# ISU-PAAL/DeepDFA

Measured on NVIDIA H100. Metric: CFG graphs/sec (train step), higher is better.
Workload: dtype f32 (GRU GEMMs: bf16x3 split operands, f32 accumulate)

## Files before the change

### deepdfa_b200/_lib.py

```python
from __future__ import annotations

import ctypes as C
import os
import re
from pathlib import Path

from . import build as _build

HEADER = Path(__file__).resolve().parent.parent / "include" / "ddfa_b200.h"

ENGINE_SIMT = 0
ENGINE_TCGEN05 = 1


class DdfaError(RuntimeError):
    pass


def declared_symbols():
    text = HEADER.read_text()
    text = re.sub(r"/\*.*?\*/", "", text, flags=re.S)
    return sorted(set(re.findall(r"\b(ddfa_[a-z0-9_]+)\s*\(", text)))


# ... 34 lines not shown
    "ddfa_gru_step_fwd_image_v2": (_int, [_vp, _vp, _vp, _vp, _i32, _i32, _vp, _vp, _vp, _vp, _sz, _vp]),
    "ddfa_gru_step_bwd_image_v2": (_int, [_vp] * 9 + [_i32, _i32] + [_vp] * 7 + [_vp, _sz, _int, _vp]),
    "ddfa_gru_step_bwd_image": (_int, [_vp] * 9 + [_i32, _i32] + [_vp] * 7 + [_vp, _sz, _int, _vp]),
    "ddfa_gru_step_bwd_finish": (_int, [_i32, _i32, _vp, _vp, _vp, _sz, _vp]),
    "ddfa_gru_step_bwd_workspace_bytes": (_sz, [_i32, _i32, _int]),
    "ddfa_gru_step_bwd_workspace_bytes_steps": (_sz, [_i32, _i32, _int, _i32]),
    "ddfa_gru_bwd_wgrad_batched": (_int, [_vp, _vp, _i32, _i32, _i32, _vp, _vp, _vp, _sz, _vp]),
    "ddfa_gru_step_prepare_bwd": (_int, [_vp, _vp, _i32, _int, _vp, _sz, _vp]),
    "ddfa_gru_step_bwd": (_int, [_vp] * 7 + [_i32, _i32] + [_vp] * 7 + [_vp, _sz, _int, _vp]),
    "ddfa_ggnn_workspace_bytes": (_sz, [_i32, _i32, _i32, _int, _int]),
    "ddfa_ggnn_fwd": (_int, [_vp, _vp, _vp, _i32, _i32, _i32] + [_vp] * 7 + [_vp, _sz, _int, _int, _vp]),
    "ddfa_ggnn_bwd": (_int, [_vp, _vp, _vp, _vp, _i32, _i32, _i32] + [_vp] * 12 + [_vp, _sz, _int, _vp]),
    "ddfa_readout_mlp_fwd": (_int, [_vp, _vp, _vp, _i32, _i32, _vp, _vp, _vp, _vp, _i32] + [_vp] * 6 + [_vp]),
    "ddfa_mlp_bwd": (_int, [_vp, _vp, _vp, _vp, _i32, _i32, _i32, _vp, _vp, _vp, _vp, _vp]),
    "ddfa_readout_bwd": (_int, [_vp] * 5 + [_i32, _i32] + [_vp] * 8 + [_vp]),
    "ddfa_graph_label_bce": (_int, [_vp, _vp, _vp, _i32, _f32, _f32, _f32, _vp, _vp, _vp, _vp]),
    "ddfa_graph_label_bce_valid": (_int, [_vp, _vp, _vp, _i32, _i32, _f32, _f32, _f32, _vp, _vp, _vp, _vp]),
    "ddfa_adam_flat": (_int, [_vp, _vp, _vp, _vp, _vp, _i64, _f32, _f32, _f32, _f32, _f32, _vp]),
    "ddfa_allreduce_adam_p2p": (_int, [_vp, _vp, _vp, _i32, _i32, _vp, _vp, _vp, _i64, _i64, _vp, _vp, _f32, _f32, _f32, _f32, _f32, _vp]),
    "ddfa_sgemm": (_int, [_int, _int, _i32, _i32, _i32, _f32, _vp, _i32, _vp, _i32, _f32, _vp, _i32, _i32, _vp]),
}

TUNE_L2_HINTS, TUNE_PDL_MASK, TUNE_GATHER_VARIANT, TUNE_FWD_PAIR, TUNE_GATE_BWD_TMA, TUNE_GATHER_SRC_GROUPS = 0, 1, 2, 3, 4, 5

_NO_STATUS = {"ddfa_gru_gates_packed_bytes", "ddfa_tuning_get", "ddfa_abi_version", "ddfa_last_error", "ddfa_device_supported", "ddfa_launch_count", "ddfa_engine_available",
              "ddfa_build_csr_workspace_bytes", "ddfa_arena_batch_workspace_bytes", "ddfa_gru_step_workspace_bytes", "ddfa_gru_step_bwd_workspace_bytes", "ddfa_gru_step_bwd_workspace_bytes_steps",
              "ddfa_act_image_bytes", "ddfa_ggnn_workspace_bytes"}


class _Lib:
    def __init__(self):
        path = Path(os.environ["DDFA_LIB_PATH"]) if os.environ.get("DDFA_LIB_PATH") else _build.LIB
        if not path.exists():
            raise DdfaError(
                f"{path} is missing: build it with `python -m deepdfa_b200.build` (or __graft_entry__.build()). "
                "deepdfa_b200 has no CPU / PyTorch fallback.")
        self.path = path
        self._dll = C.CDLL(str(path))
        missing = []
        for name, (res, args) in _SIGNATURES.items():
            try:
                fn = getattr(self._dll, name)
            except AttributeError:
                missing.append(name)
                continue
            fn.restype = res
            fn.argtypes = args
        if missing:
            raise DdfaError(f"{path} does not export: {missing}")
        abi = self._dll.ddfa_abi_version()
        if abi != 1:
            raise DdfaError(f"ABI version mismatch: library {abi}, binding 1")
        for env, key in (("DDFA_L2_HINTS", TUNE_L2_HINTS), ("DDFA_PDL", TUNE_PDL_MASK), ("DDFA_GATHER_VARIANT", TUNE_GATHER_VARIANT),
                         ("DDFA_GATE_BWD_TMA", TUNE_GATE_BWD_TMA),
                         ("DDFA_GATHER_SRC_GROUPS", TUNE_GATHER_SRC_GROUPS)):
            if os.environ.get(env) is not None:
                self._dll.ddfa_tuning_set(key, int(os.environ[env]))

    def last_error(self) -> str:
        msg = self._dll.ddfa_last_error()
        return msg.decode() if msg else ""

    def raw(self, name):
        return getattr(self._dll, name)

    def call(self, name, *args):
        rc = getattr(self._dll, name)(*args)
        if name not in _NO_STATUS and rc != 0:
            raise DdfaError(f"{name} failed (status {rc}): {self.last_error()}")
        return rc


_LIB = None


def lib() -> _Lib:
    global _LIB
    if _LIB is None:
# ... 8 lines not shown
```

### deepdfa_b200/csrc/abi.cu

```cuda
#include <stdarg.h>
#include <stdlib.h>
#include <string.h>

#include <atomic>

#include "common.cuh"

namespace ddfa {
static std::atomic<long long> g_launches{0};
void count_launch() { g_launches.fetch_add(1, std::memory_order_relaxed); }

static thread_local char g_err[512] = "";

static thread_local bool g_chain_break = true;
void chain_break() { g_chain_break = true; }
bool chain_take_break() {
  const bool b = g_chain_break;
  g_chain_break = false;
  return b;
}

static std::atomic<int> g_tuning[DDFA_TUNE__COUNT] = {
    {23},
    {15},
    {9},
    {0},
    {2},
    {0},
};
int l2_hints() { return g_tuning[DDFA_TUNE_L2_HINTS].load(std::memory_order_relaxed); }
int pdl_mask() { return g_tuning[DDFA_TUNE_PDL_MASK].load(std::memory_order_relaxed); }
int gather_variant() { return g_tuning[DDFA_TUNE_GATHER_VARIANT].load(std::memory_order_relaxed); }
int gate_bwd_tma() { return g_tuning[DDFA_TUNE_GATE_BWD_TMA].load(std::memory_order_relaxed); }
int gather_src_groups() { return g_tuning[DDFA_TUNE_GATHER_SRC_GROUPS].load(std::memory_order_relaxed); }

void set_error(const char *fmt, ...) {
  va_list ap;
  va_start(ap, fmt);
  vsnprintf(g_err, sizeof(g_err), fmt, ap);
  va_end(ap);
}
}

extern "C" {

int ddfa_abi_version(void) { return DDFA_ABI_VERSION; }

const char *ddfa_last_error(void) { return ddfa::g_err; }

int ddfa_engine_available(int engine) {
  if (engine == DDFA_ENGINE_SIMT) return 1;
  if (engine == DDFA_ENGINE_TCGEN05) return 1;
  return 0;
}

int ddfa_tuning_set(int key, int value) {
  DDFA_REQUIRE(key >= 0 && key < DDFA_TUNE__COUNT, "ddfa_tuning_set: unknown key %d", key);
  DDFA_REQUIRE(key != DDFA_TUNE_FWD_PAIR || value == 0, "ddfa_tuning_set: DDFA_TUNE_FWD_PAIR must be 0 (no CTA-pair forward kernel on sm_90a)");
  ddfa::g_tuning[key].store(value, std::memory_order_relaxed);
  return DDFA_OK;
}
int ddfa_tuning_get(int key) {
  if (key < 0 || key >= DDFA_TUNE__COUNT) return -1;
  return ddfa::g_tuning[key].load(std::memory_order_relaxed);
}

int ddfa_debug_set(int key, int value) {
  switch (key) {
    case 2: {
      int rc = ddfa::gru_tc3_trace_enable(value);
      return rc != DDFA_OK ? rc : ddfa::gru_tc2b_trace_enable(value);
    }
    default: ddfa::set_error("ddfa_debug_set: unknown key %d", key); return DDFA_ERR_INVALID_ARG;
  }
}

int ddfa_debug_read(int key, void *host_out, size_t bytes) {
  DDFA_REQUIRE(host_out != nullptr, "ddfa_debug_read: null output");
  switch (key) {
    case 2: return ddfa::gru_tc2b_trace_read(host_out, bytes);
    case 3: return ddfa::gru_tc3_trace_read(host_out, bytes);
// ... 23 lines not shown
```

### deepdfa_b200/csrc/common.cuh

```cuda
#pragma once
#include <cuda_runtime.h>
#include <stdint.h>
#include <stdio.h>

#include "../../include/ddfa_b200.h"

namespace ddfa {

void set_error(const char *fmt, ...);
void count_launch();

inline cudaStream_t as_stream(void *s) { return reinterpret_cast<cudaStream_t>(s); }

#define DDFA_REQUIRE(cond, ...)            \
  do {                                     \
    if (!(cond)) {                         \
      ddfa::set_error(__VA_ARGS__);        \
      return DDFA_ERR_INVALID_ARG;         \
    }                                      \
  } while (0)

#define DDFA_CHECK_LAUNCH(name)                                                        \
  do {                                                                                 \
    cudaError_t e__ = cudaGetLastError();                                              \
// ... 1 lines not shown
      ddfa::set_error("%s: launch failed: %s", name, cudaGetErrorString(e__));         \
      return DDFA_ERR_CUDA;                                                            \
    }                                                                                  \
    ddfa::count_launch();                                                              \
  } while (0)

#define DDFA_CUDA(call)                                                                \
  do {                                                                                 \
    cudaError_t e__ = (call);                                                          \
    if (e__ != cudaSuccess) {                                                          \
      ddfa::set_error("%s failed: %s", #call, cudaGetErrorString(e__));                \
      return DDFA_ERR_CUDA;                                                            \
    }                                                                                  \
  } while (0)

__device__ __forceinline__ void pdl_launch_dependents() { asm volatile("griddepcontrol.launch_dependents;" ::: "memory"); }
__device__ __forceinline__ void pdl_wait() { asm volatile("griddepcontrol.wait;" ::: "memory"); }
int pdl_mask();
int gather_variant();
int gather_src_groups();
int gate_bwd_tma();
void chain_break();
bool chain_take_break();

template <typename... KArgs, typename... Args>
inline cudaError_t launch_chain_cluster(int which, int cluster_x, void (*kernel)(KArgs...), dim3 grid, dim3 block, size_t smem,
                                        cudaStream_t stream, Args... args) {
  cudaLaunchConfig_t cfg = {};
  cfg.gridDim = grid;
  cfg.blockDim = block;
  cfg.dynamicSmemBytes = smem;
  cfg.stream = stream;
  cudaLaunchAttribute attr[2];
  int n = 0;
  if (cluster_x > 1) {
    attr[n].id = cudaLaunchAttributeClusterDimension;
    attr[n].val.clusterDim.x = (unsigned)cluster_x;
    attr[n].val.clusterDim.y = 1;
    attr[n].val.clusterDim.z = 1;
    ++n;
  }
  const bool brk = chain_take_break();
  if ((pdl_mask() & which) && !brk) {
    attr[n].id = cudaLaunchAttributeProgrammaticStreamSerialization;
    attr[n].val.programmaticStreamSerializationAllowed = 1;
    ++n;
// ... 131 lines not shown
```

### deepdfa_b200/csrc/gru_tc_bwd.cu

```cuda
#include <cuda_fp16.h>

#include "tc_common.cuh"

namespace ddfa {
namespace tc2b {
using namespace tcc;

constexpr int kThreads = 320, kEpiWarps = 8;

constexpr int kGbWarps = 8;
struct GbRow {
  float4 d, hv, rr, zz, nn, gh;
  float deg;
  int tb, te;
};
__device__ __forceinline__ float4 bf16x4_to_f4(const uint2 &p) {
  return make_float4(__uint_as_float(p.x << 16), __uint_as_float(p.x & 0xffff0000u), __uint_as_float(p.y << 16), __uint_as_float(p.y & 0xffff0000u));
}
__device__ __forceinline__ void gb_load(GbRow &x, const float *__restrict__ dh_out, const float *__restrict__ h,
                                        const uint8_t *__restrict__ h_img_src, const float *__restrict__ gates,
                                        const uint4 *__restrict__ gates_packed, const int32_t *__restrict__ indptr,
                                        const int32_t *__restrict__ indptr_t, size_t plane, int64_t node, int col, bool ok,
                                        uint64_t pol_saved, uint64_t pol_dh) {
  x.tb = x.te = 0;
// ... 465 lines not shown
        }
      }
    }
    wgmma_wait<0>();
    wgmma_fence_regs(acc);
    if (tr) { trace_stamp(tron, k, 6); trace_stamp(tron, k, 8); }
    __syncwarp();
    if (lane == 0) mbar_arrive(empty(pending));
    pending = -1;
    if (tr) trace_stamp(tron, k, 9);
#pragma unroll
    for (int hh = 0; hh < 2; ++hh) {
      const int64_t node = (int64_t)tile * kTileM + row0 + 8 * hh;
      if (node < N) {
#pragma unroll
        for (int j = 0; j < 8; ++j)
          st_f2_hint(out + node * kD + col0 + 8 * j, make_float2(acc[4 * j + 2 * hh] + dv[hh][j].x, acc[4 * j + 2 * hh + 1] + dv[hh][j].y), pol_tmp);
      }
    }
    if (tr) trace_stamp(tron, k, 10);
  }
}

constexpr int kWgSlotBytes = kImageTileBytes;
constexpr int kWgSlots = 3;
constexpr int kWgOffBar = kWgSlots * kWgSlotBytes;
constexpr int kWgSmemAlloc = kWgOffBar + 2 * kWgSlots * 8 + 1024;
constexpr int kWgThreads = 32 * kEpiWarps + 32;
constexpr size_t kWgPartialFloats = (size_t)3 * kD * kD;
constexpr int kWgMaxSteps = 16;
struct WgBatch {
  const uint8_t *s_img[kWgMaxSteps];
  const uint8_t *h_img[kWgMaxSteps];
  int32_t steps;
};
__global__ void __launch_bounds__(kWgThreads, 1) wgrad_kernel(const uint8_t *__restrict__ q_img, size_t img_stride, size_t step_stride,
                                                              const __grid_constant__ WgBatch batch,
                                                              int32_t N, float *__restrict__ partial, int first, int hints) {
  extern __shared__ uint8_t smem_raw[];
  uint8_t *smem = reinterpret_cast<uint8_t *>((reinterpret_cast<uintptr_t>(smem_raw) + 1023) & ~(uintptr_t)1023);
  const uint32_t sbase = smem_u32(smem);
  const uint32_t bar0 = sbase + kWgOffBar;
  auto full = [&](int i) { return bar0 + 8u * i; };
  auto empty = [&](int i) { return bar0 + 8u * (kWgSlots + i); };

  const int warp = threadIdx.x >> 5, lane = threadIdx.x & 31;
  const int role = blockIdx.y / 3, g = blockIdx.y % 3;
  const int qm = g < 2 ? g : (role == 0 ? 2 : 3);
  const int num_tiles = (N + kTileM - 1) / kTileM;
  const int all_tiles = num_tiles * batch.steps;
  const int my_tiles = (all_tiles > (int)blockIdx.x) ? (all_tiles - 1 - (int)blockIdx.x) / (int)gridDim.x + 1 : 0;

  if (threadIdx.x == 0) {
    for (int i = 0; i < kWgSlots; ++i) { mbar_init(full(i), 1); mbar_init(empty(i), kEpiWarps); }
    mbar_fence_init();
  }
  __syncthreads();
  const int tron = (g_trace_on == 2) && blockIdx.y == 0;
  if (threadIdx.x == 0) trace_stamp(tron, 0, 0);

  if (warp == kEpiWarps) {
    if (elect_one()) {
      const uint64_t pol_wg = l2_policy((hints & 32) ? 1 : 0);
      for (int i = 0; i < my_tiles; ++i) {
        const int idx = (int)blockIdx.x + i * (int)gridDim.x;
        const int t = idx / num_tiles, tile = idx - t * num_tiles;
        for (int w = 0; w < 2; ++w) {
          const int cc = 2 * i + w, slot = cc % kWgSlots, use = cc / kWgSlots;
          if (use > 0) mbar_wait_bounded(empty(slot), (use - 1) & 1);
          const uint8_t *src = w == 0 ? (role == 0 ? batch.s_img[t] : batch.h_img[t]) : q_img + (size_t)t * step_stride + (size_t)qm * img_stride;
          mbar_arrive_expect_tx(full(slot), kWgSlotBytes);
          bulk_g2s_hint(sbase + slot * kWgSlotBytes, src + (size_t)tile * kImageTileBytes, kWgSlotBytes, full(slot), pol_wg);
          trace_stamp(tron, i, 1 + w);
        }
      }
    }
    return;
  }

  const int wg = warp >> 2;
  float acc[64];
#pragma unroll
  for (int i = 0; i < 64; ++i) acc[i] = 0.f;
  for (int i = 0; i < my_tiles; ++i) {
    const int cb = 2 * i, ca = 2 * i + 1;
    mbar_wait_bounded(full(cb % kWgSlots), (cb / kWgSlots) & 1);
    if (warp == 0 && lane == 0) trace_stamp(tron, i, 3);
    mbar_wait_bounded(full(ca % kWgSlots), (ca / kWgSlots) & 1);
    if (warp == 0 && lane == 0) { trace_stamp(tron, i, 4); trace_stamp(tron, i, 5); }
    const uint32_t b0 = sbase + (cb % kWgSlots) * kWgSlotBytes;
    const uint32_t a0 = sbase + (ca % kWgSlots) * kWgSlotBytes + wg * kChunkBytes;
    constexpr uint32_t vs = 2 * kChunkBytes;
    wgmma_fence();
#pragma unroll
    for (int k16 = 0; k16 < kTileM / 16; ++k16) {
      const uint32_t koff = (uint32_t)k16 * 2048u;
      const uint64_t a_hi = gmma_desc(a0 + koff, kChunkBytes), a_lo = gmma_desc(a0 + vs + koff, kChunkBytes);
      const uint64_t b_hi = gmma_desc(b0 + koff, kChunkBytes), b_lo = gmma_desc(b0 + vs + koff, kChunkBytes);
      wgmma_n128<1, 1>(acc, a_hi, b_hi, 1u);
      wgmma_n128<1, 1>(acc, a_lo, b_hi, 1u);
      wgmma_n128<1, 1>(acc, a_hi, b_lo, 1u);
    }
    wgmma_commit();
    if (warp == 0 && lane == 0) trace_stamp(tron, i, 6);
    wgmma_wait<0>();
    __syncwarp();
    if (lane == 0) { mbar_arrive(empty(cb % kWgSlots)); mbar_arrive(empty(ca % kWgSlots)); }
  }
  wgmma_fence_regs(acc);
  if (warp == 0 && lane == 0) trace_stamp(tron, 0, 8);
  float *dst = partial + ((size_t)role * gridDim.x + blockIdx.x) * kWgPartialFloats;
  const int row0 = g * kD + wg * 64 + (warp & 3) * 16 + (lane >> 2);
#pragma unroll
  for (int hh = 0; hh < 2; ++hh) {
    float *rowp = dst + (size_t)(row0 + 8 * hh) * kD + 2 * (lane & 3);
#pragma unroll
    for (int j = 0; j < 16; ++j) {
      float2 v = make_float2(acc[4 * j + 2 * hh], acc[4 * j + 2 * hh + 1]);
      if (!first) {
        const float2 o = *reinterpret_cast<const float2 *>(rowp + 8 * j);
        v.x += o.x;
        v.y += o.y;
      }
      *reinterpret_cast<float2 *>(rowp + 8 * j) = v;
    }
  }
  if (warp == 0 && lane == 0) trace_stamp(tron, 0, 10);
}

__global__ void __launch_bounds__(256) wgrad_reduce_kernel(const float *__restrict__ partial, int ctas, float *__restrict__ dw_fold,
                                                           float *__restrict__ dw_hh) {
// ... 155 lines not shown
```

### deepdfa_b200/csrc/gru_tc_fwd3.cu

```cuda
#include <cuda_fp16.h>
#include <stdlib.h>

#include "tc_common.cuh"

namespace ddfa {
namespace tc3 {
using namespace tcc;

constexpr int kSlices = 4;
constexpr int kSliceCols = kD / kSlices;
constexpr int kRowsPerPart = 3 * kSliceCols;
constexpr int kWChunkBytes = kRowsPerPart * 128;
constexpr int kSliceWBytes = 8 * kWChunkBytes;
constexpr int kStageBytes = kImageTileBytes;
constexpr int kOffStage = kSliceWBytes;
constexpr int kOffBias = kOffStage + 2 * kStageBytes;
constexpr int kBiasSlice = 7 * kSliceCols;
constexpr int kOffBar = kOffBias + kBiasSlice * 4;
constexpr int kSmemAlloc = kOffBar + 5 * 8;
constexpr int kConsumerWarps = 8;
constexpr int kThreads = 32 * kConsumerWarps + 32;
constexpr size_t kPackedWBytes = (size_t)kSlices * kSliceWBytes;
constexpr size_t kPackedBytes = kPackedWBytes + (size_t)kSlices * kBiasSlice * 4;
static_assert(kSmemAlloc <= 232448, "shared memory budget");
// ... 11 lines not shown
  uint4 ph, pl;
  split8(x, ph, pl);
  uint8_t *base = packed + (size_t)slice * kSliceWBytes + sw128_offset(n, (u & 7) * 8);
  *reinterpret_cast<uint4 *>(base + ((p * 2 + 0) * 2 + kb) * kWChunkBytes) = ph;
  *reinterpret_cast<uint4 *>(base + ((p * 2 + 1) * 2 + kb) * kWChunkBytes) = pl;
  if (p == 0 && u == 0 && n < kSliceCols) {
    const int t = slice * kSliceCols + n;
    float *bias = reinterpret_cast<float *>(packed + kPackedWBytes) + slice * kBiasSlice;
    bias[0 * kSliceCols + n] = b_ih[2 * kD + t];
    bias[1 * kSliceCols + n] = b_ih[t] + b_hh[t];
    bias[2 * kSliceCols + n] = b_ih[kD + t] + b_hh[kD + t];
    bias[3 * kSliceCols + n] = b_hh[2 * kD + t];
    bias[4 * kSliceCols + n] = b_fold[2 * kD + t];
    bias[5 * kSliceCols + n] = b_fold[t];
    bias[6 * kSliceCols + n] = b_fold[kD + t];
  }
}

template <bool HIMG, int GATES>
__global__ void __launch_bounds__(kThreads, 1) gru_fwd3_kernel(const uint8_t *__restrict__ s_img, const uint8_t *__restrict__ h_img,
                                                               const float *__restrict__ h, const int32_t *__restrict__ indptr,
                                                               const uint8_t *__restrict__ packed, int32_t N,
                                                               float *__restrict__ h_out, uint8_t *__restrict__ h_out_img,
                                                               float *__restrict__ gates, uint2 *__restrict__ gates_packed, int hints) {
  extern __shared__ __align__(1024) uint8_t smem[];
  const uint32_t sbase = smem_u32(smem);
  if ((sbase & 1023u) != 0) __trap();
  const uint32_t bar0 = sbase + kOffBar;
  auto full = [&](int i) { return bar0 + 8u * i; };
  auto empty = [&](int i) { return bar0 + 8u * (2 + i); };
  const uint32_t w_full = bar0 + 32u;

  const int warp = threadIdx.x >> 5, lane = threadIdx.x & 31;
  const int slice = blockIdx.x % kSlices;
  const int group = blockIdx.x / kSlices, num_groups = gridDim.x / kSlices;
  const int num_tiles = (N + kTileM - 1) / kTileM;
  const int my_tiles = (num_tiles > group) ? (num_tiles - 1 - group) / num_groups + 1 : 0;

  if (threadIdx.x == 0) {
    for (int i = 0; i < 2; ++i) { mbar_init(full(i), 1); mbar_init(empty(i), kConsumerWarps); }
    mbar_init(w_full, 1);
    mbar_fence_init();
  }
  __syncthreads();
  const int tron = g_trace_on;
  if (threadIdx.x == 0) trace_stamp(tron, 0, 0);
  pdl_launch_dependents();

  if (warp == kConsumerWarps) {
    if (my_tiles > 0 && elect_one()) {
      mbar_arrive_expect_tx(w_full, kSliceWBytes);
      bulk_g2s(sbase, packed + (size_t)slice * kSliceWBytes, kSliceWBytes, w_full);
      pdl_wait();
      for (int k = 0; k < my_tiles; ++k) {
        const size_t toff = (size_t)(group + k * num_groups) * kImageTileBytes;
        for (int p = 0; p < 2; ++p) {
          if (k > 0) mbar_wait_bounded(empty(p), (k - 1) & 1);
          mbar_arrive_expect_tx(full(p), kStageBytes);
          bulk_g2s(sbase + kOffStage + p * kStageBytes, (p == 0 ? s_img : h_img) + toff, kStageBytes, full(p));
          trace_stamp(tron, k, 1 + p);
        }
      }
    }
    return;
  }

  float *sbias = reinterpret_cast<float *>(smem + kOffBias);
  for (int i = threadIdx.x; i < kBiasSlice; i += 32 * kConsumerWarps)
    sbias[i] = __ldcg(reinterpret_cast<const float *>(packed + kPackedWBytes) + slice * kBiasSlice + i);
  asm volatile("bar.sync 1, %0;" ::"n"(32 * kConsumerWarps) : "memory");
  pdl_wait();
  if (my_tiles == 0) return;
  const int wg = warp >> 2;
  const int row0 = wg * 64 + (warp & 3) * 16 + (lane >> 2);
  const int c4 = 2 * (lane & 3);
  const size_t plane = (size_t)N * kD;
  const uint64_t pol_gates = l2_policy((hints & 1) ? 1 : 0);
  const uint64_t pol_next = l2_policy((hints & 16) ? 2 : 0);
  mbar_wait_bounded(w_full, 0);
  const bool tr = (warp == 0 && lane == 0);

  for (int k = 0; k < my_tiles; ++k) {
    const int tile = group + k * num_groups;
    float acc_s[48], acc_h[48];
    if (tr) { trace_stamp(tron, k, 7); trace_stamp(tron, k, 3); }
    mbar_wait_bounded(full(0), k & 1);
    if (tr) trace_stamp(tron, k, 4);
    wgmma_fence();
#pragma unroll
    for (int p = 0; p < 2; ++p) {
      if (p == 1) {
        mbar_wait_bounded(full(1), k & 1);
        if (tr) trace_stamp(tron, k, 5);
      }
      const uint32_t a0 = sbase + kOffStage + p * kStageBytes + wg * 8192;
// ... 24 lines not shown
      const int64_t node = (int64_t)tile * kTileM + row0 + 8 * hh;
      const bool valid = node < N;
      deg[hh] = valid ? (float)(__ldcg(indptr + node + 1) - __ldcg(indptr + node)) : 0.f;
#pragma unroll
      for (int j = 0; j < 4; ++j) {
        const int gcol = slice * kSliceCols + 8 * j + c4;
        if constexpr (HIMG) {
          const uint32_t whi = __ldcg(reinterpret_cast<const uint32_t *>(h_img + image_offset(node, gcol, 0)));
          const uint32_t wlo = __ldcg(reinterpret_cast<const uint32_t *>(h_img + image_offset(node, gcol, 1)));
          hp[hh][2 * j] = __uint_as_float(whi << 16) + __uint_as_float(wlo << 16);
          hp[hh][2 * j + 1] = __uint_as_float(whi & 0xffff0000u) + __uint_as_float(wlo & 0xffff0000u);
        } else {
          const float2 v = valid ? __ldcg(reinterpret_cast<const float2 *>(h + node * kD + gcol)) : make_float2(0.f, 0.f);
          hp[hh][2 * j] = v.x;
          hp[hh][2 * j + 1] = v.y;
        }
      }
    }
    wgmma_wait<0>();
    wgmma_fence_regs(acc_s);
    wgmma_fence_regs(acc_h);
    if (tr) { trace_stamp(tron, k, 6); trace_stamp(tron, k, 8); }
    __syncwarp();
    if (lane == 0) { mbar_arrive(empty(0)); mbar_arrive(empty(1)); }
    if (tr) trace_stamp(tron, k, 9);

#pragma unroll
    for (int hh = 0; hh < 2; ++hh) {
      const int64_t node = (int64_t)tile * kTileM + row0 + 8 * hh;
      const bool valid = node < N;
#pragma unroll
      for (int j = 0; j < 4; ++j) {
        const int c = 8 * j + c4, gcol = slice * kSliceCols + c;
        float hn[2], rr[2], zz[2], nn[2], gg[2];
#pragma unroll
        for (int e = 0; e < 2; ++e) {
          const int i = 2 * hh + e;
          const float dg = deg[hh];
          const float gin = acc_s[4 * (8 + j) + i] + fmaf(dg, sbias[4 * kSliceCols + c + e], sbias[c + e]);
          const float r = fast_sigmoid(acc_s[4 * j + i] + acc_h[4 * j + i] + fmaf(dg, sbias[5 * kSliceCols + c + e], sbias[kSliceCols + c + e]));
          const float z = fast_sigmoid(acc_s[4 * (4 + j) + i] + acc_h[4 * (4 + j) + i] +
                                       fmaf(dg, sbias[6 * kSliceCols + c + e], sbias[2 * kSliceCols + c + e]));
          const float ghn = acc_h[4 * (8 + j) + i] + sbias[3 * kSliceCols + c + e];
          const float n = fast_tanh(fmaf(r, ghn, gin));
          hn[e] = valid ? fmaf(z, hp[hh][2 * j + e] - n, n) : 0.f;
          rr[e] = r; zz[e] = z; nn[e] = n; gg[e] = ghn;
        }
// ... 3 lines not shown
          if (valid) {
            const uint2 g0 = pack_gates(rr[0], zz[0], nn[0], gg[0]), g1 = pack_gates(rr[1], zz[1], nn[1], gg[1]);
            st_u4_hint(gates_packed + off, make_uint4(g0.x, g0.y, g1.x, g1.y), pol_gates);
          }
        }
        if constexpr (GATES == 1) {
          if (valid) {
            st_f2_hint(gates + off, make_float2(rr[0], rr[1]), pol_gates);
            st_f2_hint(gates + plane + off, make_float2(zz[0], zz[1]), pol_gates);
            st_f2_hint(gates + 2 * plane + off, make_float2(nn[0], nn[1]), pol_gates);
            st_f2_hint(gates + 3 * plane + off, make_float2(gg[0], gg[1]), pol_gates);
          }
        }
        if (h_out_img != nullptr) {
          const uint32_t hw = bf16x2_bits(hn[0], hn[1]);
          const uint32_t lw = bf16x2_bits(hn[0] - __uint_as_float(hw << 16), hn[1] - __uint_as_float(hw & 0xffff0000u));
          st_u32_hint(h_out_img + image_offset(node, gcol, 0), hw, pol_next);
          st_u32_hint(h_out_img + image_offset(node, gcol, 1), lw, pol_next);
        }
      }
    }
    if (tr) trace_stamp(tron, k, 10);
  }
}

}

size_t gru_tc3_packed_bytes() { return tc3::kPackedBytes; }

int gru_tc3_prepare(const float *w_fold, const float *b_fold, const float *b_ih, const float *w_hh, const float *b_hh, void *packed,
                    cudaStream_t stream) {
  const int total = tc3::kSlices * 2 * tc3::kRowsPerPart * 16;
  tc3::pack_kernel<<<(total + 127) / 128, 128, 0, stream>>>(w_fold, w_hh, b_fold, b_ih, b_hh, static_cast<uint8_t *>(packed));
  DDFA_CHECK_LAUNCH("tc3::pack_kernel");
  chain_break();
  return DDFA_OK;
}

int gru_tc3_step_fwd(const void *s_img, const void *h_img, const float *h, const int32_t *indptr, int32_t N, float *h_out,
                     void *h_out_img, float *save_gates, void *save_gates_packed, const void *packed, cudaStream_t stream) {
  const int tiles = (N + tcc::kTileM - 1) / tcc::kTileM;
  int groups = kNumSMs / tc3::kSlices;
  if (groups > tiles) groups = tiles;
  if (save_gates && save_gates_packed) {
    set_error("tcgen05 engine (fwd): both gate formats requested");
    return DDFA_ERR_INVALID_ARG;
  }
  if ((h == nullptr && save_gates) ) {
    set_error("tcgen05 engine (fwd): fp32 gate planes go with the fp32 h operand (legacy form)");
    return DDFA_ERR_INVALID_ARG;
  }
  if (tiles == 0) return DDFA_OK;
#define DDFA_FWD3_LAUNCH(HIMG, GATES)                                                                                                     \
  do {                                                                                                                                   \
    DDFA_CUDA(cudaFuncSetAttribute(tc3::gru_fwd3_kernel<HIMG, GATES>, cudaFuncAttributeMaxDynamicSharedMemorySize, tc3::kSmemAlloc));     \
    DDFA_CUDA(launch_chain(2, tc3::gru_fwd3_kernel<HIMG, GATES>, dim3(groups * tc3::kSlices), dim3(tc3::kThreads), tc3::kSmemAlloc,        \
                           stream, static_cast<const uint8_t *>(s_img), static_cast<const uint8_t *>(h_img), h, indptr,                   \
                           static_cast<const uint8_t *>(packed), N, h_out, static_cast<uint8_t *>(h_out_img), save_gates,                \
                           static_cast<uint2 *>(save_gates_packed), l2_hints()));                                                        \
  } while (0)
  if (h) {
    if (save_gates) DDFA_FWD3_LAUNCH(false, 1);
    else if (save_gates_packed) DDFA_FWD3_LAUNCH(false, 2);
    else DDFA_FWD3_LAUNCH(false, 0);
  } else {
    if (save_gates_packed) DDFA_FWD3_LAUNCH(true, 2);
    else DDFA_FWD3_LAUNCH(true, 0);
  }
#undef DDFA_FWD3_LAUNCH
  DDFA_CHECK_LAUNCH("tc3::gru_fwd3_kernel");
  return DDFA_OK;
}

namespace tc3 {
__global__ void __launch_bounds__(256) to_image_kernel(const float *__restrict__ x, int32_t N, uint8_t *__restrict__ image) {
  const int64_t t = blockIdx.x * (int64_t)blockDim.x + threadIdx.x;
  const int64_t rows = ((int64_t)N + kTileM - 1) / kTileM * kTileM;
  if (t >= rows * 16) return;
  const int64_t node = t >> 4;
  const int col = (int)(t & 15) * 8;
  float v[8] = {0.f, 0.f, 0.f, 0.f, 0.f, 0.f, 0.f, 0.f};
  if (node < N) {
// ... 54 lines not shown
```

### deepdfa_b200/csrc/tc_common.cuh

```cuda
#pragma once
#include <cuda_bf16.h>

#include "common.cuh"

namespace ddfa {
namespace tcc {

constexpr int kD = 128;
constexpr int kTileM = 128;
constexpr int kChunkBytes = 128 * 128;
constexpr int kImageTileBytes = 4 * kChunkBytes;

__host__ __device__ __forceinline__ size_t image_bytes(int64_t n) { return (size_t)((n + kTileM - 1) / kTileM) * kImageTileBytes; }

__device__ __forceinline__ uint32_t smem_u32(const void *p) { return (uint32_t)__cvta_generic_to_shared(p); }

__device__ __forceinline__ void mbar_init(uint32_t bar, uint32_t count) {
  asm volatile("mbarrier.init.shared::cta.b64 [%0], %1;" ::"r"(bar), "r"(count));
}
__device__ __forceinline__ void mbar_fence_init() { asm volatile("fence.mbarrier_init.release.cluster;" ::: "memory"); }
__device__ __forceinline__ void mbar_arrive(uint32_t bar) {
  asm volatile("mbarrier.arrive.shared::cta.b64 _, [%0];" ::"r"(bar) : "memory");
}
__device__ __forceinline__ void mbar_arrive_expect_tx(uint32_t bar, uint32_t bytes) {
// ... 15 lines not shown
__device__ __forceinline__ void bulk_g2s(uint32_t dst, const void *src, uint32_t bytes, uint32_t bar) {
  asm volatile("cp.async.bulk.shared::cluster.global.mbarrier::complete_tx::bytes [%0], [%1], %2, [%3];" ::"r"(dst), "l"(src),
               "r"(bytes), "r"(bar)
               : "memory");
}
__device__ __forceinline__ bool elect_one() {
  uint32_t pred = 0;
  asm volatile(
      "{\n"
      ".reg .b32 rx;\n"
      ".reg .pred px;\n"
      "elect.sync rx|px, 0xffffffff;\n"
      "@px mov.s32 %0, 1;\n"
      "}\n"
      : "+r"(pred));
  return pred != 0;
}
__device__ __forceinline__ uint64_t desc_advance(uint64_t desc, uint32_t byte_off) { return desc + (uint64_t)(byte_off >> 4); }

__device__ __forceinline__ void bulk_g2s_hint(uint32_t dst, const void *src, uint32_t bytes, uint32_t bar, uint64_t pol) {
  asm volatile("cp.async.bulk.shared::cluster.global.mbarrier::complete_tx::bytes.L2::cache_hint [%0], [%1], %2, [%3], %4;" ::"r"(dst),
               "l"(src), "r"(bytes), "r"(bar), "l"(pol)
               : "memory");
}

__device__ __forceinline__ uint64_t gmma_desc(uint32_t saddr, uint32_t lbo_bytes = 16u) {
  return (uint64_t)((saddr & 0x3FFFFu) >> 4) | ((uint64_t)((lbo_bytes >> 4) & 0x3FFFu) << 16) | ((uint64_t)(1024 >> 4) << 32) |
         ((uint64_t)1 << 62);
}
__device__ __forceinline__ void wgmma_fence() { asm volatile("wgmma.fence.sync.aligned;" ::: "memory"); }
__device__ __forceinline__ void wgmma_commit() { asm volatile("wgmma.commit_group.sync.aligned;" ::: "memory"); }
template <int N>
__device__ __forceinline__ void wgmma_wait() { asm volatile("wgmma.wait_group.sync.aligned %0;" ::"n"(N) : "memory"); }
template <int R>
__device__ __forceinline__ void wgmma_fence_regs(float (&d)[R]) {
#pragma unroll
  for (int i = 0; i < R; ++i) asm volatile("" : "+f"(d[i])::"memory");
}

template <int TA, int TB>
__device__ __forceinline__ void wgmma_n64(float (&d)[32], uint64_t a, uint64_t b, uint32_t accumulate) {
  asm volatile(
      "{\n.reg .pred p;\nsetp.ne.b32 p, %34, 0;\n"
      "wgmma.mma_async.sync.aligned.m64n64k16.f32.bf16.bf16 {%0, %1, %2, %3, %4, %5, %6, %7, %8, %9, %10, %11, %12, %13, %14, %15, %16, %17, %18, %19, %20, %21, %22, %23, %24, %25, %26, %27, %28, %29, %30, %31}, %32, %33, p, 1, 1, %35, %36;\n}\n"
      : "+f"(d[0]), "+f"(d[1]), "+f"(d[2]), "+f"(d[3]), "+f"(d[4]), "+f"(d[5]), "+f"(d[6]), "+f"(d[7]), "+f"(d[8]), "+f"(d[9]), "+f"(d[10]), "+f"(d[11]), "+f"(d[12]), "+f"(d[13]), "+f"(d[14]), "+f"(d[15]), "+f"(d[16]), "+f"(d[17]), "+f"(d[18]), "+f"(d[19]), "+f"(d[20]), "+f"(d[21]), "+f"(d[22]), "+f"(d[23]), "+f"(d[24]), "+f"(d[25]), "+f"(d[26]), "+f"(d[27]), "+f"(d[28]), "+f"(d[29]), "+f"(d[30]), "+f"(d[31])
      : "l"(a), "l"(b), "r"(accumulate), "n"(TA), "n"(TB));
// ... 114 lines not shown
```

### include/ddfa_b200.h

```cpp
#ifndef DDFA_B200_H
#define DDFA_B200_H

#include <stddef.h>
#include <stdint.h>

#ifdef __cplusplus
extern "C" {
#endif

#define DDFA_ABI_VERSION 1

typedef enum ddfa_status {
  DDFA_OK = 0,
  DDFA_ERR_INVALID_ARG = -1,
  DDFA_ERR_CUDA = -2,
  DDFA_ERR_UNSUPPORTED = -3,
  DDFA_ERR_WORKSPACE = -4
} ddfa_status;

#define DDFA_ENGINE_SIMT 0
#define DDFA_ENGINE_TCGEN05 1

int ddfa_abi_version(void);
const char *ddfa_last_error(void);
int ddfa_device_supported(void);
int ddfa_engine_available(int engine);
enum {
  DDFA_TUNE_L2_HINTS = 0,
  DDFA_TUNE_PDL_MASK = 1,
  DDFA_TUNE_GATHER_VARIANT = 2,
  DDFA_TUNE_FWD_PAIR = 3,
  DDFA_TUNE_GATE_BWD_TMA = 4,
  DDFA_TUNE_GATHER_SRC_GROUPS = 5,
  DDFA_TUNE__COUNT = 6
};
int ddfa_tuning_set(int key, int value);
int ddfa_tuning_get(int key);
int ddfa_debug_set(int key, int value);
int ddfa_debug_read(int key, void *host_out, size_t bytes);
long long ddfa_launch_count(void);


size_t ddfa_build_csr_workspace_bytes(int64_t num_edges, int32_t num_nodes);
int ddfa_build_csr(const void *src, const void *dst, int idx_bytes, int64_t num_edges,
                   int32_t num_nodes, int32_t *indptr, int32_t *indices, int32_t *indptr_t,
                   int32_t *indices_t, void *workspace, size_t workspace_bytes, void *stream);

int ddfa_graph_ptr(const int64_t *batch_num_nodes, int32_t num_graphs, int32_t *graph_ptr,
                   void *stream);

size_t ddfa_arena_batch_workspace_bytes(int32_t batch_size);
int ddfa_arena_batch(const int32_t *graph_ids, int32_t batch_size, int32_t num_graphs, const int32_t *node_off,
                     const int32_t *indptr, const int32_t *indices, const int32_t *indptr_t, const int32_t *indices_t,
                     const int64_t *const *feats, int32_t num_feats, const int32_t *vuln, int32_t batch_nodes,
                     int32_t batch_edges, int32_t *out_graph_ptr, int32_t *out_indptr, int32_t *out_indices,
                     int32_t *out_indptr_t, int32_t *out_indices_t, int64_t *const *out_feats, int32_t *out_vuln,
                     void *workspace, size_t workspace_bytes, void *stream);
// ... 124 lines not shown
```

Before: 92190.

## Pipeline GRU weight-grad loads in half-chunks and add optional cluster multicast forward

The backward weight-gradient kernel now splits each tile into half-K chunks across six smaller slots and waits on one outstanding wgmma group instead of zero. This lets TMA loads and tensor-core MMAs overlap more deeply than with three full-tile slots. The forward GRU kernel gains an optional cluster mode that multicasts the shared s/h image tiles to every CTA in a cluster, with remote empty-barrier arrivals and cluster syncs. That mode defaults to cluster size 1, so by default only the restructured backward pipeline changes behaviour. The extra chunked bulk copies raise issue overhead, and the deferred slot release adds ordering complexity.

```diff
diff --git a/deepdfa_b200/_lib.py b/deepdfa_b200/_lib.py
--- a/deepdfa_b200/_lib.py
+++ b/deepdfa_b200/_lib.py
@@ -80,6 +80,7 @@
 }
 
 TUNE_L2_HINTS, TUNE_PDL_MASK, TUNE_GATHER_VARIANT, TUNE_FWD_PAIR, TUNE_GATE_BWD_TMA, TUNE_GATHER_SRC_GROUPS = 0, 1, 2, 3, 4, 5
+TUNE_FWD_CLUSTER = 6
 
 _NO_STATUS = {"ddfa_gru_gates_packed_bytes", "ddfa_tuning_get", "ddfa_abi_version", "ddfa_last_error", "ddfa_device_supported", "ddfa_launch_count", "ddfa_engine_available",
               "ddfa_build_csr_workspace_bytes", "ddfa_arena_batch_workspace_bytes", "ddfa_gru_step_workspace_bytes", "ddfa_gru_step_bwd_workspace_bytes", "ddfa_gru_step_bwd_workspace_bytes_steps",
@@ -111,7 +112,7 @@
             raise DdfaError(f"ABI version mismatch: library {abi}, binding 1")
         for env, key in (("DDFA_L2_HINTS", TUNE_L2_HINTS), ("DDFA_PDL", TUNE_PDL_MASK), ("DDFA_GATHER_VARIANT", TUNE_GATHER_VARIANT),
                          ("DDFA_GATE_BWD_TMA", TUNE_GATE_BWD_TMA),
-                         ("DDFA_GATHER_SRC_GROUPS", TUNE_GATHER_SRC_GROUPS)):
+                         ("DDFA_GATHER_SRC_GROUPS", TUNE_GATHER_SRC_GROUPS), ("DDFA_FWD_CLUSTER", TUNE_FWD_CLUSTER)):
             if os.environ.get(env) is not None:
                 self._dll.ddfa_tuning_set(key, int(os.environ[env]))
 
diff --git a/deepdfa_b200/csrc/abi.cu b/deepdfa_b200/csrc/abi.cu
--- a/deepdfa_b200/csrc/abi.cu
+++ b/deepdfa_b200/csrc/abi.cu
@@ -3,6 +3,9 @@
 #include <string.h>
 
 #include <atomic>
+#include <map>
+#include <mutex>
+#include <utility>
 
 #include "common.cuh"
 
@@ -27,12 +30,41 @@
     {0},
     {2},
     {0},
+    {1},
 };
 int l2_hints() { return g_tuning[DDFA_TUNE_L2_HINTS].load(std::memory_order_relaxed); }
 int pdl_mask() { return g_tuning[DDFA_TUNE_PDL_MASK].load(std::memory_order_relaxed); }
 int gather_variant() { return g_tuning[DDFA_TUNE_GATHER_VARIANT].load(std::memory_order_relaxed); }
 int gate_bwd_tma() { return g_tuning[DDFA_TUNE_GATE_BWD_TMA].load(std::memory_order_relaxed); }
 int gather_src_groups() { return g_tuning[DDFA_TUNE_GATHER_SRC_GROUPS].load(std::memory_order_relaxed); }
+int fwd_cluster() { return g_tuning[DDFA_TUNE_FWD_CLUSTER].load(std::memory_order_relaxed); }
+
+int max_active_clusters(const void *kernel, int cluster_x, int block, int smem) {
+  static std::mutex mu;
+  static std::map<std::pair<const void *, int>, int> cache;
+  const auto key = std::make_pair(kernel, cluster_x);
+  std::lock_guard<std::mutex> lock(mu);
+  const auto it = cache.find(key);
+  if (it != cache.end()) return it->second;
+  cudaLaunchConfig_t cfg = {};
+  cfg.gridDim = dim3((unsigned)cluster_x);
+  cfg.blockDim = dim3((unsigned)block);
+  cfg.dynamicSmemBytes = (size_t)smem;
+  cudaLaunchAttribute attr;
+  attr.id = cudaLaunchAttributeClusterDimension;
+  attr.val.clusterDim.x = (unsigned)cluster_x;
+  attr.val.clusterDim.y = 1;
+  attr.val.clusterDim.z = 1;
+  cfg.attrs = &attr;
+  cfg.numAttrs = 1;
+  int n = 0;
+  if (cudaOccupancyMaxActiveClusters(&n, kernel, &cfg) != cudaSuccess) {
+    cudaGetLastError();
+    n = 0;
+  }
+  cache[key] = n;
+  return n;
+}
 
 void set_error(const char *fmt, ...) {
   va_list ap;
@@ -57,6 +89,7 @@
 int ddfa_tuning_set(int key, int value) {
   DDFA_REQUIRE(key >= 0 && key < DDFA_TUNE__COUNT, "ddfa_tuning_set: unknown key %d", key);
   DDFA_REQUIRE(key != DDFA_TUNE_FWD_PAIR || value == 0, "ddfa_tuning_set: DDFA_TUNE_FWD_PAIR must be 0 (no CTA-pair forward kernel on sm_90a)");
+  DDFA_REQUIRE(key != DDFA_TUNE_FWD_CLUSTER || value == 1 || value == 2 || value == 4, "ddfa_tuning_set: DDFA_TUNE_FWD_CLUSTER must be 1, 2 or 4 (got %d)", value);
   ddfa::g_tuning[key].store(value, std::memory_order_relaxed);
   return DDFA_OK;
 }
diff --git a/deepdfa_b200/csrc/common.cuh b/deepdfa_b200/csrc/common.cuh
--- a/deepdfa_b200/csrc/common.cuh
+++ b/deepdfa_b200/csrc/common.cuh
@@ -47,6 +47,9 @@
 int gate_bwd_tma();
 void chain_break();
 bool chain_take_break();
+
+int fwd_cluster();
+int max_active_clusters(const void *kernel, int cluster_x, int block, int smem);
 
 template <typename... KArgs, typename... Args>
 inline cudaError_t launch_chain_cluster(int which, int cluster_x, void (*kernel)(KArgs...), dim3 grid, dim3 block, size_t smem,
diff --git a/deepdfa_b200/csrc/gru_tc_bwd.cu b/deepdfa_b200/csrc/gru_tc_bwd.cu
--- a/deepdfa_b200/csrc/gru_tc_bwd.cu
+++ b/deepdfa_b200/csrc/gru_tc_bwd.cu
@@ -511,8 +511,9 @@
   }
 }
 
-constexpr int kWgSlotBytes = kImageTileBytes;
-constexpr int kWgSlots = 3;
+constexpr int kWgHalfChunk = kChunkBytes / 2;
+constexpr int kWgSlotBytes = 4 * kWgHalfChunk;
+constexpr int kWgSlots = 6;
 constexpr int kWgOffBar = kWgSlots * kWgSlotBytes;
 constexpr int kWgSmemAlloc = kWgOffBar + 2 * kWgSlots * 8 + 1024;
 constexpr int kWgThreads = 32 * kEpiWarps + 32;
@@ -551,16 +552,20 @@
   if (warp == kEpiWarps) {
     if (elect_one()) {
       const uint64_t pol_wg = l2_policy((hints & 32) ? 1 : 0);
-      for (int i = 0; i < my_tiles; ++i) {
+      for (int hi = 0; hi < 2 * my_tiles; ++hi) {
+        const int i = hi >> 1, half = hi & 1;
         const int idx = (int)blockIdx.x + i * (int)gridDim.x;
         const int t = idx / num_tiles, tile = idx - t * num_tiles;
         for (int w = 0; w < 2; ++w) {
-          const int cc = 2 * i + w, slot = cc % kWgSlots, use = cc / kWgSlots;
+          const int cc = 2 * hi + w, slot = cc % kWgSlots, use = cc / kWgSlots;
           if (use > 0) mbar_wait_bounded(empty(slot), (use - 1) & 1);
-          const uint8_t *src = w == 0 ? (role == 0 ? batch.s_img[t] : batch.h_img[t]) : q_img + (size_t)t * step_stride + (size_t)qm * img_stride;
+          const uint8_t *src = (w == 0 ? (role == 0 ? batch.s_img[t] : batch.h_img[t]) : q_img + (size_t)t * step_stride + (size_t)qm * img_stride) +
+                               (size_t)tile * kImageTileBytes + half * kWgHalfChunk;
           mbar_arrive_expect_tx(full(slot), kWgSlotBytes);
-          bulk_g2s_hint(sbase + slot * kWgSlotBytes, src + (size_t)tile * kImageTileBytes, kWgSlotBytes, full(slot), pol_wg);
-          trace_stamp(tron, i, 1 + w);
+#pragma unroll
+          for (int c = 0; c < 4; ++c)
+            bulk_g2s_hint(sbase + slot * kWgSlotBytes + c * kWgHalfChunk, src + c * kChunkBytes, kWgHalfChunk, full(slot), pol_wg);
+          if (half == 0) trace_stamp(tron, i, 1 + w);
         }
       }
     }
@@ -571,31 +576,34 @@
   float acc[64];
 #pragma unroll
   for (int i = 0; i < 64; ++i) acc[i] = 0.f;
-  for (int i = 0; i < my_tiles; ++i) {
-    const int cb = 2 * i, ca = 2 * i + 1;
+  for (int hi = 0; hi < 2 * my_tiles; ++hi) {
+    const int i = hi >> 1, half = hi & 1;
+    const int cb = 2 * hi, ca = 2 * hi + 1;
+    const bool tr = warp == 0 && lane == 0 && half == 0;
     mbar_wait_bounded(full(cb % kWgSlots), (cb / kWgSlots) & 1);
-    if (warp == 0 && lane == 0) trace_stamp(tron, i, 3);
+    if (tr) trace_stamp(tron, i, 3);
     mbar_wait_bounded(full(ca % kWgSlots), (ca / kWgSlots) & 1);
-    if (warp == 0 && lane == 0) { trace_stamp(tron, i, 4); trace_stamp(tron, i, 5); }
+    if (tr) { trace_stamp(tron, i, 4); trace_stamp(tron, i, 5); }
     const uint32_t b0 = sbase + (cb % kWgSlots) * kWgSlotBytes;
-    const uint32_t a0 = sbase + (ca % kWgSlots) * kWgSlotBytes + wg * kChunkBytes;
-    constexpr uint32_t vs = 2 * kChunkBytes;
+    const uint32_t a0 = sbase + (ca % kWgSlots) * kWgSlotBytes + wg * kWgHalfChunk;
+    constexpr uint32_t vs = 2 * kWgHalfChunk;
     wgmma_fence();
 #pragma unroll
-    for (int k16 = 0; k16 < kTileM / 16; ++k16) {
+    for (int k16 = 0; k16 < kTileM / 32; ++k16) {
       const uint32_t koff = (uint32_t)k16 * 2048u;
-      const uint64_t a_hi = gmma_desc(a0 + koff, kChunkBytes), a_lo = gmma_desc(a0 + vs + koff, kChunkBytes);
-      const uint64_t b_hi = gmma_desc(b0 + koff, kChunkBytes), b_lo = gmma_desc(b0 + vs + koff, kChunkBytes);
+      const uint64_t a_hi = gmma_desc(a0 + koff, kWgHalfChunk), a_lo = gmma_desc(a0 + vs + koff, kWgHalfChunk);
+      const uint64_t b_hi = gmma_desc(b0 + koff, kWgHalfChunk), b_lo = gmma_desc(b0 + vs + koff, kWgHalfChunk);
       wgmma_n128<1, 1>(acc, a_hi, b_hi, 1u);
       wgmma_n128<1, 1>(acc, a_lo, b_hi, 1u);
       wgmma_n128<1, 1>(acc, a_hi, b_lo, 1u);
     }
     wgmma_commit();
-    if (warp == 0 && lane == 0) trace_stamp(tron, i, 6);
-    wgmma_wait<0>();
+    if (warp == 0 && lane == 0 && half == 1) trace_stamp(tron, i, 6);
+    wgmma_wait<1>();
     __syncwarp();
-    if (lane == 0) { mbar_arrive(empty(cb % kWgSlots)); mbar_arrive(empty(ca % kWgSlots)); }
-  }
+    if (hi > 0 && lane == 0) { mbar_arrive(empty((cb - 2) % kWgSlots)); mbar_arrive(empty((ca - 2) % kWgSlots)); }
+  }
+  wgmma_wait<0>();
   wgmma_fence_regs(acc);
   if (warp == 0 && lane == 0) trace_stamp(tron, 0, 8);
   float *dst = partial + ((size_t)role * gridDim.x + blockIdx.x) * kWgPartialFloats;
diff --git a/deepdfa_b200/csrc/gru_tc_fwd3.cu b/deepdfa_b200/csrc/gru_tc_fwd3.cu
--- a/deepdfa_b200/csrc/gru_tc_fwd3.cu
+++ b/deepdfa_b200/csrc/gru_tc_fwd3.cu
@@ -57,7 +57,8 @@
                                                                const float *__restrict__ h, const int32_t *__restrict__ indptr,
                                                                const uint8_t *__restrict__ packed, int32_t N,
                                                                float *__restrict__ h_out, uint8_t *__restrict__ h_out_img,
-                                                               float *__restrict__ gates, uint2 *__restrict__ gates_packed, int hints) {
+                                                               float *__restrict__ gates, uint2 *__restrict__ gates_packed, int hints,
+                                                               int cluster) {
   extern __shared__ __align__(1024) uint8_t smem[];
   const uint32_t sbase = smem_u32(smem);
   if ((sbase & 1023u) != 0) __trap();
@@ -71,32 +72,43 @@
   const int group = blockIdx.x / kSlices, num_groups = gridDim.x / kSlices;
   const int num_tiles = (N + kTileM - 1) / kTileM;
   const int my_tiles = (num_tiles > group) ? (num_tiles - 1 - group) / num_groups + 1 : 0;
+  const uint32_t crank = (uint32_t)(slice % cluster);
+  const uint16_t cmask = (uint16_t)((1u << cluster) - 1u);
 
   if (threadIdx.x == 0) {
-    for (int i = 0; i < 2; ++i) { mbar_init(full(i), 1); mbar_init(empty(i), kConsumerWarps); }
+    for (int i = 0; i < 2; ++i) { mbar_init(full(i), 1); mbar_init(empty(i), kConsumerWarps * cluster); }
     mbar_init(w_full, 1);
     mbar_fence_init();
   }
-  __syncthreads();
+  if (cluster > 1) cluster_sync();
+  else __syncthreads();
+  if (my_tiles == 0) return;
   const int tron = g_trace_on;
   if (threadIdx.x == 0) trace_stamp(tron, 0, 0);
   pdl_launch_dependents();
 
   if (warp == kConsumerWarps) {
-    if (my_tiles > 0 && elect_one()) {
+    if (elect_one()) {
       mbar_arrive_expect_tx(w_full, kSliceWBytes);
       bulk_g2s(sbase, packed + (size_t)slice * kSliceWBytes, kSliceWBytes, w_full);
       pdl_wait();
       for (int k = 0; k < my_tiles; ++k) {
         const size_t toff = (size_t)(group + k * num_groups) * kImageTileBytes;
         for (int p = 0; p < 2; ++p) {
-          if (k > 0) mbar_wait_bounded(empty(p), (k - 1) & 1);
+          const bool issuer = crank == (uint32_t)(p % cluster);
+          if (k > 0) mbar_wait_bounded(issuer ? empty(p) : full(p), (k - 1) & 1);
           mbar_arrive_expect_tx(full(p), kStageBytes);
-          bulk_g2s(sbase + kOffStage + p * kStageBytes, (p == 0 ? s_img : h_img) + toff, kStageBytes, full(p));
+          if (issuer) {
+            const uint8_t *src = (p == 0 ? s_img : h_img) + toff;
+            if (cluster > 1) bulk_g2s_multicast(sbase + kOffStage + p * kStageBytes, src, kStageBytes, full(p), cmask, l2_policy(0));
+            else bulk_g2s(sbase + kOffStage + p * kStageBytes, src, kStageBytes, full(p));
+          }
           trace_stamp(tron, k, 1 + p);
         }
       }
     }
+    __syncwarp();
+    if (cluster > 1) cluster_sync();
     return;
   }
 
@@ -105,7 +117,6 @@
     sbias[i] = __ldcg(reinterpret_cast<const float *>(packed + kPackedWBytes) + slice * kBiasSlice + i);
   asm volatile("bar.sync 1, %0;" ::"n"(32 * kConsumerWarps) : "memory");
   pdl_wait();
-  if (my_tiles == 0) return;
   const int wg = warp >> 2;
   const int row0 = wg * 64 + (warp & 3) * 16 + (lane >> 2);
   const int c4 = 2 * (lane & 3);
@@ -176,7 +187,10 @@
     wgmma_fence_regs(acc_h);
     if (tr) { trace_stamp(tron, k, 6); trace_stamp(tron, k, 8); }
     __syncwarp();
-    if (lane == 0) { mbar_arrive(empty(0)); mbar_arrive(empty(1)); }
+    if (lane == 0) {
+      if (cluster > 1) { mbar_arrive_cluster(empty(0), 0); mbar_arrive_cluster(empty(1), 1 % cluster); }
+      else { mbar_arrive(empty(0)); mbar_arrive(empty(1)); }
+    }
     if (tr) trace_stamp(tron, k, 9);
 
 #pragma unroll
@@ -226,6 +240,7 @@
     }
     if (tr) trace_stamp(tron, k, 10);
   }
+  if (cluster > 1) cluster_sync();
 }
 
 }
@@ -244,8 +259,7 @@
 int gru_tc3_step_fwd(const void *s_img, const void *h_img, const float *h, const int32_t *indptr, int32_t N, float *h_out,
                      void *h_out_img, float *save_gates, void *save_gates_packed, const void *packed, cudaStream_t stream) {
   const int tiles = (N + tcc::kTileM - 1) / tcc::kTileM;
-  int groups = kNumSMs / tc3::kSlices;
-  if (groups > tiles) groups = tiles;
+  const int cluster = fwd_cluster();
   if (save_gates && save_gates_packed) {
     set_error("tcgen05 engine (fwd): both gate formats requested");
     return DDFA_ERR_INVALID_ARG;
@@ -258,10 +272,20 @@
 #define DDFA_FWD3_LAUNCH(HIMG, GATES)                                                                                                     \
   do {                                                                                                                                   \
     DDFA_CUDA(cudaFuncSetAttribute(tc3::gru_fwd3_kernel<HIMG, GATES>, cudaFuncAttributeMaxDynamicSharedMemorySize, tc3::kSmemAlloc));     \
-    DDFA_CUDA(launch_chain(2, tc3::gru_fwd3_kernel<HIMG, GATES>, dim3(groups * tc3::kSlices), dim3(tc3::kThreads), tc3::kSmemAlloc,        \
-                           stream, static_cast<const uint8_t *>(s_img), static_cast<const uint8_t *>(h_img), h, indptr,                   \
-                           static_cast<const uint8_t *>(packed), N, h_out, static_cast<uint8_t *>(h_out_img), save_gates,                \
-                           static_cast<uint2 *>(save_gates_packed), l2_hints()));                                                        \
+    int groups = kNumSMs / tc3::kSlices;                                                                                                 \
+    if (cluster > 1) {                                                                                                                   \
+      const int mac = max_active_clusters((const void *)tc3::gru_fwd3_kernel<HIMG, GATES>, cluster, tc3::kThreads, tc3::kSmemAlloc); \
+      if (mac * cluster / tc3::kSlices < groups) groups = mac * cluster / tc3::kSlices;                                                  \
+      if (groups < 1) {                                                                                                                  \
+        set_error("tcgen05 engine (fwd): clusters of %d CTAs cannot be resident", cluster);                                         \
+        return DDFA_ERR_CUDA;                                                                                                            \
+      }                                                                                                                                  \
+    }                                                                                                                                    \
+    if (groups > tiles) groups = tiles;                                                                                                  \
+    DDFA_CUDA(launch_chain_cluster(2, cluster, tc3::gru_fwd3_kernel<HIMG, GATES>, dim3(groups * tc3::kSlices), dim3(tc3::kThreads), \
+                                   tc3::kSmemAlloc, stream, static_cast<const uint8_t *>(s_img), static_cast<const uint8_t *>(h_img), h, \
+                                   indptr, static_cast<const uint8_t *>(packed), N, h_out, static_cast<uint8_t *>(h_out_img), save_gates, \
+                                   static_cast<uint2 *>(save_gates_packed), l2_hints(), cluster));                                        \
   } while (0)
   if (h) {
     if (save_gates) DDFA_FWD3_LAUNCH(false, 1);
diff --git a/deepdfa_b200/csrc/tc_common.cuh b/deepdfa_b200/csrc/tc_common.cuh
--- a/deepdfa_b200/csrc/tc_common.cuh
+++ b/deepdfa_b200/csrc/tc_common.cuh
@@ -61,6 +61,22 @@
   asm volatile("cp.async.bulk.shared::cluster.global.mbarrier::complete_tx::bytes.L2::cache_hint [%0], [%1], %2, [%3], %4;" ::"r"(dst),
                "l"(src), "r"(bytes), "r"(bar), "l"(pol)
                : "memory");
+}
+
+__device__ __forceinline__ void bulk_g2s_multicast(uint32_t dst, const void *src, uint32_t bytes, uint32_t bar, uint16_t cta_mask,
+                                                   uint64_t pol) {
+  asm volatile(
+      "cp.async.bulk.shared::cluster.global.mbarrier::complete_tx::bytes.multicast::cluster.L2::cache_hint [%0], [%1], %2, [%3], %4, %5;" ::"r"(dst),
+      "l"(src), "r"(bytes), "r"(bar), "h"(cta_mask), "l"(pol)
+      : "memory");
+}
+__device__ __forceinline__ void mbar_arrive_cluster(uint32_t bar, uint32_t rank) {
+  uint32_t remote;
+  asm volatile("mapa.shared::cluster.u32 %0, %1, %2;" : "=r"(remote) : "r"(bar), "r"(rank));
+  asm volatile("mbarrier.arrive.release.cluster.shared::cluster.b64 _, [%0];" ::"r"(remote) : "memory");
+}
+__device__ __forceinline__ void cluster_sync() {
+  asm volatile("barrier.cluster.arrive.release;\nbarrier.cluster.wait.acquire;" ::: "memory");
 }
 
 __device__ __forceinline__ uint64_t gmma_desc(uint32_t saddr, uint32_t lbo_bytes = 16u) {
diff --git a/include/ddfa_b200.h b/include/ddfa_b200.h
--- a/include/ddfa_b200.h
+++ b/include/ddfa_b200.h
@@ -32,7 +32,8 @@
   DDFA_TUNE_FWD_PAIR = 3,
   DDFA_TUNE_GATE_BWD_TMA = 4,
   DDFA_TUNE_GATHER_SRC_GROUPS = 5,
-  DDFA_TUNE__COUNT = 6
+  DDFA_TUNE_FWD_CLUSTER = 6,
+  DDFA_TUNE__COUNT = 7
 };
 int ddfa_tuning_set(int key, int value);
 int ddfa_tuning_get(int key);
```

After: 92180, median of 6. No clear change (-0.0%).
